# borglab/gtsfm

Measured on NVIDIA H100. Metric: image_pairs_per_sec, higher is better.
Workload: dtype f32

## Files before the change

### gtsfm_b200/csrc/gemm_ws.cuh

```cuda
#pragma once
#include "tma.cuh"

constexpr int GW_MAXP = 16;
constexpr int GW_M = 128, GW_N = 128, GW_K = 64;
constexpr int GW_A_BYTES = GW_M * GW_K * 2;
constexpr int GW_B_BYTES = GW_N * GW_K * 2;
constexpr int GW_STAGE_BYTES = 2 * GW_A_BYTES + 2 * GW_B_BYTES;
constexpr int GW_STAGES = 2;
constexpr int GW_PITCH = GW_N + 8;
constexpr int GW_STG_BYTES = GW_M * GW_PITCH * 4;
constexpr int GW_RB = 8;
constexpr int GW_EW = 4;
constexpr int GW_THREADS = 512;
constexpr size_t GW_SMEM = GW_STAGES * GW_STAGE_BYTES + GW_STG_BYTES + 1024  + 256 ;
constexpr int GW_SEGS = 3;

struct GemmProblem {
  const float* resid;
  float* C;
  __half *Ch[GW_SEGS], *Cl[GW_SEGS];
  const float *cs, *sn;
  int M, N, ldc;
  int vec4;
  int tiles_n;
  int tile_end;
};
struct GemmWsMaps {
  CUtensorMap a1h[GW_MAXP], a1l[GW_MAXP];
  CUtensorMap a2h[GW_MAXP], a2l[GW_MAXP];
  CUtensorMap bh[GW_MAXP], bl[GW_MAXP];
};
struct GemmWsArgs {
  GemmProblem p[GW_MAXP];
  int nprob, tiles;
  int K1, K2;
  int b_per_problem;
  const float* bias;
  int ldr;
  float scale;
  int ldch;
  int head_major;
  int relu;
  int gelu;
  int lo_unscaled;
  int seg_n;
  int rot_mask;
  int* err_flag;
};

static __device__ __noinline__ float gelu_erf(float x) { return 0.5f * x * (1.0f + erff(x * 0.70710678118654752440f)); }

static __global__ void __launch_bounds__(GW_THREADS, 1) k_gemm_ws(const __grid_constant__ GemmWsMaps maps, const __grid_constant__ GemmWsArgs g) {
  extern __shared__ unsigned char gw_raw[];
  const uint32_t raw = tc::smem_u32(gw_raw);
  const uint32_t smem0 = (raw + 1023u) & ~1023u;
  unsigned char* sm = gw_raw + (smem0 - raw);
  float* stg = reinterpret_cast<float*>(sm + GW_STAGES * GW_STAGE_BYTES);
  uint64_t* full = reinterpret_cast<uint64_t*>(sm + GW_STAGES * GW_STAGE_BYTES + GW_STG_BYTES);
  uint64_t* empty = full + GW_STAGES;
  uint64_t* sfull = empty + GW_STAGES;
  uint64_t* sempty = sfull + 1;

  const int t = threadIdx.x, warp = t >> 5, lane = t & 31;
  const int nk = (g.K1 + g.K2) / GW_K;

  if (t == 0) {
    for (int s = 0; s < GW_STAGES; ++s) tc::mbar_init(&full[s], 1), tc::mbar_init(&empty[s], 8);
    tc::mbar_init(sfull, 256);
    tc::mbar_init(sempty, 32 * GW_EW);
    tc::fence_mbar_init();
    tc::tma_prefetch_desc(&maps.bh[0]);
    tc::tma_prefetch_desc(&maps.bl[0]);
  }
  __syncthreads();
  bool ok = true;

  auto decode = [&](int tile, int& z, int& m0, int& n0) {
    z = 0;
    while (z + 1 < g.nprob && tile >= g.p[z].tile_end) ++z;
    const int local = tile - (z ? g.p[z - 1].tile_end : 0);
    const int mt = local / g.p[z].tiles_n;
    n0 = (local - mt * g.p[z].tiles_n) * GW_N;
    m0 = mt * GW_M;
  };

  if (warp >= 12) {
    asm volatile("setmaxnreg.dec.sync.aligned.u32 40;\n" ::: "memory");
    if (warp == 12 && lane == 0) {
      int gk = 0;
      for (int tile = blockIdx.x; tile < g.tiles; tile += gridDim.x) {
        int z, m0, n0;
        decode(tile, z, m0, n0);
        const int zb = g.b_per_problem ? z : 0;
        for (int kc = 0; kc < nk; ++kc, ++gk) {
          const int s = gk % GW_STAGES;
          if (gk >= GW_STAGES) ok = tc::mbar_wait(&empty[s], ((gk / GW_STAGES) - 1) & 1) && ok;
          const int k0 = kc * GW_K;
          const bool seg2 = k0 >= g.K1;
          const CUtensorMap* ah = seg2 ? &maps.a2h[z] : &maps.a1h[z];
          const CUtensorMap* al = seg2 ? &maps.a2l[z] : &maps.a1l[z];
          const int ka = seg2 ? k0 - g.K1 : k0;
          const uint32_t sA = smem0 + s * GW_STAGE_BYTES, sB = sA + 2 * GW_A_BYTES;
          tc::mbar_expect_tx(&full[s], GW_STAGE_BYTES);
          tc::tma_load_2d(sA, ah, &full[s], ka, m0);
          tc::tma_load_2d(sA + GW_A_BYTES, al, &full[s], ka, m0);
          tc::tma_load_2d(sB, &maps.bh[zb], &full[s], k0, n0);
          tc::tma_load_2d(sB + GW_B_BYTES, &maps.bl[zb], &full[s], k0, n0);
        }
      }
    }
  } else if (warp < 8) {
    asm volatile("setmaxnreg.inc.sync.aligned.u32 184;\n" ::: "memory");
    const int wg = warp >> 2;
    const int r0 = wg * 64 + (warp & 3) * 16 + (lane >> 2);
    const int c2 = (lane & 3) * 2;
    int gk = 0, it = 0;
    for (int tile = blockIdx.x; tile < g.tiles; tile += gridDim.x, ++it) {
      float acc0[64], acc1[64];
      for (int kc = 0; kc < nk; ++kc, ++gk) {
        const int s = gk % GW_STAGES;
        ok = tc::mbar_wait(&full[s], (gk / GW_STAGES) & 1) && ok;
        const uint32_t aH = smem0 + s * GW_STAGE_BYTES + wg * (64 * 128), aL = aH + GW_A_BYTES;
        const uint32_t bH = smem0 + s * GW_STAGE_BYTES + 2 * GW_A_BYTES, bL = bH + GW_B_BYTES;
        const uint64_t dAh = tc::wg_desc_sw128(aH), dAl = tc::wg_desc_sw128(aL), dBh = tc::wg_desc_sw128(bH), dBl = tc::wg_desc_sw128(bL);
        tc::wg_fence();
#pragma unroll
        for (int ks = 0; ks < GW_K / 16; ++ks) {
          const uint64_t adv = (uint64_t)(ks * 2);
          const uint32_t first = (kc == 0 && ks == 0) ? 0u : 1u;
          tc::wg_ss_n128(acc0, dAh + adv, dBh + adv, first);
          tc::wg_ss_n128(acc1, dAh + adv, dBl + adv, first);
          tc::wg_ss_n128(acc1, dAl + adv, dBh + adv, 1u);
        }
        tc::wg_commit();
        if (kc > 0) {
          tc::wg_wait<1>();
          if (lane == 0) tc::mbar_arrive(&empty[(gk - 1) % GW_STAGES]);
        }
      }
      tc::wg_wait<0>();
      if (lane == 0) tc::mbar_arrive(&empty[(gk - 1) % GW_STAGES]);

      if (it > 0) ok = tc::mbar_wait(sempty, (it - 1) & 1) && ok;
#pragma unroll
      for (int j = 0; j < 16; ++j)
#pragma unroll
        for (int h = 0; h < 2; ++h) {
          const int i = 4 * j + 2 * h;
          *reinterpret_cast<float2*>(stg + (r0 + 8 * h) * GW_PITCH + 8 * j + c2) =
              make_float2(fmaf(acc1[i], tc::LO_INV, acc0[i]), fmaf(acc1[i + 1], tc::LO_INV, acc0[i + 1]));
        }
      tc::mbar_arrive(sfull);
    }
  } else {
    asm volatile("setmaxnreg.dec.sync.aligned.u32 104;\n" ::: "memory");
    const int ew = warp - 8;
    const int c = 4 * lane;
    const float scale = g.scale;
    const int relu = g.relu, gelu = g.gelu, hm = g.head_major, lo_unscaled = g.lo_unscaled, ldr = g.ldr, ldch = g.ldch;
    int it = 0;
    for (int tile = blockIdx.x; tile < g.tiles; tile += gridDim.x, ++it) {
      int z, m0, n0;
      decode(tile, z, m0, n0);
      const GemmProblem& pb = g.p[z];
      const float* resid = pb.resid;
      float* C = pb.C;
      const int sg = g.seg_n ? n0 / g.seg_n : 0;
      __half *Ch = pb.Ch[sg], *Cl = pb.Cl[sg];
      const bool rot = (g.rot_mask >> sg) & 1;
      const int M = pb.M, ldc = pb.ldc;
      const int n = n0 + c;
      const int ncols = min(4, pb.N - n);
      const bool vec = pb.vec4 && ncols == 4;
      const int rows = min(GW_M, M - m0);
      float b4[4] = {0.f, 0.f, 0.f, 0.f};
      if (g.bias)
#pragma unroll
        for (int e = 0; e < 4; ++e)
          if (e < ncols) b4[e] = __ldg(g.bias + n + e);
      const int ns = n - sg * g.seg_n;
      const size_t hm_col = (size_t)(ns >> 6) * M * 64 + (ns & 63);
      const bool vres = resid && vec;
      const int rp = (ns & 63) >> 1;
      float4 rr[GW_RB];
      auto load_rows = [&](int rb) {
        if (rot) {
#pragma unroll
          for (int i = 0; i < GW_RB; ++i)
            if (rb + GW_EW * i < rows) {
              const size_t o = (size_t)(m0 + rb + GW_EW * i) * 32 + rp;
              const float2 cc = __ldg(reinterpret_cast<const float2*>(pb.cs + o)), ss = __ldg(reinterpret_cast<const float2*>(pb.sn + o));
              rr[i] = make_float4(cc.x, cc.y, ss.x, ss.y);
            }
        } else {
#pragma unroll
          for (int i = 0; i < GW_RB; ++i)
            if (rb + GW_EW * i < rows) rr[i] = *reinterpret_cast<const float4*>(resid + (size_t)(m0 + rb + GW_EW * i) * ldr + n);
        }
      };
      if (vres || rot) load_rows(ew);
      ok = tc::mbar_wait(sfull, it & 1) && ok;
      auto pre = [&](int r, float* v) {
        const float4 a = *reinterpret_cast<const float4*>(stg + r * GW_PITCH + c);
        v[0] = a.x, v[1] = a.y, v[2] = a.z, v[3] = a.w;
#pragma unroll
        for (int e = 0; e < 4; ++e) {
          v[e] = (v[e] + b4[e]) * scale;
          if (relu) v[e] = fmaxf(v[e], 0.f);
          if (gelu) v[e] = gelu_erf(v[e]);
        }
      };
      if (ncols > 0 && vec) {
        for (int rb = ew; rb < rows; rb += GW_EW * GW_RB) {
          if ((vres || rot) && rb != ew) load_rows(rb);
#pragma unroll
          for (int i = 0; i < GW_RB; ++i) {
            const int r = rb + GW_EW * i;
            if (r >= rows) break;
            const int row = m0 + r;
            float v[4];
            pre(r, v);
            if (resid) v[0] += rr[i].x, v[1] += rr[i].y, v[2] += rr[i].z, v[3] += rr[i].w;
            if (rot) {
              const float c0 = rr[i].x, c1 = rr[i].y, s0 = rr[i].z, s1 = rr[i].w;
              const float a0 = __fadd_rn(__fmul_rn(v[0], c0), __fmul_rn(-v[1], s0)), a1 = __fadd_rn(__fmul_rn(v[1], c0), __fmul_rn(v[0], s0));
              const float a2 = __fadd_rn(__fmul_rn(v[2], c1), __fmul_rn(-v[3], s1)), a3 = __fadd_rn(__fmul_rn(v[3], c1), __fmul_rn(v[2], s1));
              v[0] = a0, v[1] = a1, v[2] = a2, v[3] = a3;
            }
            const size_t off = hm ? hm_col + (size_t)row * 64 : (size_t)row * ldc + n;
            if (C) *reinterpret_cast<float4*>(C + off) = make_float4(v[0], v[1], v[2], v[3]);
            if (Ch) {
              const size_t off_s = hm ? off : (size_t)row * ldch + n;
              uint32_t h01, l01, h23, l23;
              if (lo_unscaled) {
                tc::split2_unscaled_clamped(v[0], v[1], h01, l01);
                tc::split2_unscaled_clamped(v[2], v[3], h23, l23);
              } else {
                tc::split2(v[0], v[1], h01, l01);
                tc::split2(v[2], v[3], h23, l23);
              }
              *reinterpret_cast<uint2*>(Ch + off_s) = make_uint2(h01, h23);
              *reinterpret_cast<uint2*>(Cl + off_s) = make_uint2(l01, l23);
            }
          }
        }
      } else if (ncols > 0) {
#pragma unroll 1
        for (int r = ew; r < rows; r += GW_EW) {
          const int row = m0 + r;
          float v[4];
          pre(r, v);
          const size_t off_c = hm ? hm_col + (size_t)row * 64 : (size_t)row * ldc + n;
          const size_t off_s = hm ? hm_col + (size_t)row * 64 : (size_t)row * ldch + n;
#pragma unroll
          for (int e = 0; e < 4; ++e) {
            if (e >= ncols) break;
            if (resid) v[e] += resid[(size_t)row * ldr + n + e];
            if (C) C[off_c + e] = v[e];
            if (Ch) {
              __half hh, ll;
              if (lo_unscaled) tc::split_h_unscaled(v[e], hh, ll);
              else tc::split_h(v[e], hh, ll);
              Ch[off_s + e] = hh;
              Cl[off_s + e] = ll;
            }
          }
        }
      }
      tc::mbar_arrive(sempty);
    }
  }
  if (!ok && g.err_flag) *g.err_flag = 1;
}
```

### gtsfm_b200/csrc/linear.cuh

```cuda
#pragma once
#include "attn_ps.cuh"
#include "common.cuh"
#include "gemm.cuh"
#include "gemm_ws.cuh"

struct TcWeights {
  const float* f;
  const __half* h;
  const __half* l;
  int* err;
  bool use_tc;
  DevBuf* attn_part = nullptr;
  DevBuf* attn_ml = nullptr;
  DevBuf* attn_cnt = nullptr;
  int sm_count = 132;
};

struct Pl {
  __half* hi;
  __half* lo;
};
static inline Pl planes_of(const DevBuf& b, size_t elems) { return {b.as<__half>(), b.as<__half>() + elems}; }

struct LinArgs {
  const float* a1f = nullptr;
  Pl a1p{nullptr, nullptr};
  int lda1 = 0, K1 = 0;
  const float* a2f = nullptr;
  Pl a2p{nullptr, nullptr};
  int lda2 = 0, K2 = 0;
  const float* w = nullptr;
  const float* bf = nullptr;
  Pl bp{nullptr, nullptr};
  int ldb = 0;
  const float* bias = nullptr;
  float scale = 1.f;
  const float* resid = nullptr;
  int ldr = 0;
  float* cf = nullptr;
  int ldc = 0;
  Pl cp{nullptr, nullptr};
  int ldch = 0;
  int head_major = 0;
  bool tc_want_f32 = false;
  int relu = 0;
  int gelu = 0;
  int lo_unscaled = 0;
  int M = 0, N = 0;
  int seg_n = 0;
  float* seg_f[GW_SEGS] = {};
  Pl seg_p[GW_SEGS] = {};
  int rot_mask = 0;
  const float *cs = nullptr, *sn = nullptr;
};

static int run_linear(b2_context* ctx, cudaStream_t st, const TcWeights& tw, const LinArgs* a, int np, const char* site = nullptr) {
  if (np <= 0) return B2_OK;
  if (np > GW_MAXP) return b2_fail(ctx, B2_ERR_ARG, "run_linear: too many problems in one launch");
  const LinArgs& a0 = a[0];
  const int nseg = a0.seg_n > 0 ? a0.N / a0.seg_n : 1;
  if (a0.seg_n > 0 && (a0.seg_n % GW_N || a0.N != nseg * a0.seg_n || nseg > GW_SEGS || !a0.head_major || a0.resid || a0.tc_want_f32 ||
                       (a0.rot_mask && (!a0.cs || !a0.sn))))
    return b2_fail(ctx, B2_ERR_ARG, "run_linear: column segments need N = seg_n x (<= 3), seg_n % 128 == 0, head-major planes, "
                                    "no residual or fp32 output, and a rotary table when rotary is on");
  if (!tw.use_tc) {
    if (a0.rot_mask) return b2_fail(ctx, B2_ERR_ARG, "run_linear: the rotary epilogue exists on the wgmma path only");
    for (int i = 0; i < np; ++i) {
      const LinArgs& x = a[i];
      if (x.M <= 0 || x.N <= 0) continue;
      if (x.gelu) return b2_fail(ctx, B2_ERR_ARG, "run_linear: the GELU epilogue exists on the wgmma path only");
      if (x.K1 % GB_K || x.K2 % GB_K || x.lda1 % 4 || x.lda2 % 4 || x.ldb % 4)
        return b2_fail(ctx, B2_ERR_ARG, "run_linear: the SIMT GEMM needs K1, K2 multiples of 16 and lda1, lda2, ldb multiples of 4");
    }
    for (int i = 0; i < np; ++i) {
      const LinArgs& x = a[i];
      if (x.M <= 0 || x.N <= 0) continue;
      for (int s = 0; s < nseg; ++s) {
        const int c0 = s * x.seg_n;
        GemmArgs g{};
        g.A1 = x.a1f, g.lda1 = x.lda1, g.K1 = x.K1, g.A2 = x.a2f, g.lda2 = x.lda2, g.K2 = x.K2;
        g.B = (x.w ? x.w : x.bf) + (size_t)c0 * x.ldb, g.ldb = x.ldb, g.C = x.seg_n ? x.seg_f[s] : x.cf, g.ldc = x.ldc, g.M = x.M;
        g.N = x.seg_n ? x.seg_n : x.N;
        g.bias = x.bias ? x.bias + c0 : nullptr, g.resid = x.resid, g.ldr = x.ldr, g.scale = x.scale, g.head_major = x.head_major;
        g.relu = x.relu;
        int rc = launch_gemm(ctx, st, g);
        if (rc) return rc;
      }
    }
    return B2_OK;
  }
  if (a0.K1 % GW_K || a0.K2 % GW_K) return b2_fail(ctx, B2_ERR_ARG, "run_linear: the wgmma GEMM needs K1 and K2 multiples of 64");
  if (!tma_encoder()) return b2_fail(ctx, B2_ERR_CUDA, "cuTensorMapEncodeTiled is not available (driver too old?)");
  const bool per_b = a0.w == nullptr;
  static thread_local GemmWsMaps maps;
  GemmWsArgs q{};
  double work = 0.0;
  bool ok = true;
  int nz = 0, tiles = 0;
  for (int i = 0; i < np; ++i) {
    const LinArgs& x = a[i];
    if (x.M <= 0 || x.N <= 0) continue;
    ok = ok && tma_map_2d(&maps.a1h[nz], x.a1p.hi, x.M, x.K1, x.lda1, GW_M) && tma_map_2d(&maps.a1l[nz], x.a1p.lo, x.M, x.K1, x.lda1, GW_M);
    if (x.K2 > 0)
      ok = ok && tma_map_2d(&maps.a2h[nz], x.a2p.hi, x.M, x.K2, x.lda2, GW_M) && tma_map_2d(&maps.a2l[nz], x.a2p.lo, x.M, x.K2, x.lda2, GW_M);
    if (per_b || nz == 0) {
      const __half *bh, *bl;
      if (x.w) {
        const size_t off = (size_t)(x.w - tw.f);
        bh = tw.h + off, bl = tw.l + off;
      } else {
        bh = x.bp.hi, bl = x.bp.lo;
      }
      ok = ok && tma_map_2d(&maps.bh[nz], bh, x.N, x.K1 + x.K2, x.ldb, GW_N) && tma_map_2d(&maps.bl[nz], bl, x.N, x.K1 + x.K2, x.ldb, GW_N);
    }
    GemmProblem& pr = q.p[nz];
    pr.resid = x.resid, pr.C = x.tc_want_f32 ? x.cf : nullptr, pr.M = x.M, pr.N = x.N, pr.ldc = x.ldc;
    for (int s = 0; s < GW_SEGS; ++s) {
      const Pl p = x.seg_n ? (s < nseg ? x.seg_p[s] : Pl{nullptr, nullptr}) : (s == 0 ? x.cp : Pl{nullptr, nullptr});
      pr.Ch[s] = p.hi, pr.Cl[s] = p.lo;
    }
    pr.cs = x.cs, pr.sn = x.sn;
    {
      auto al16 = [](const void* q) { return (reinterpret_cast<uintptr_t>(q) & 15) == 0; };
      auto al8 = [](const void* q) { return (reinterpret_cast<uintptr_t>(q) & 7) == 0; };
      const bool hm = x.head_major != 0;
      bool v = al16(pr.resid) && (x.ldr % 4 == 0 || !pr.resid) && al16(pr.C) && (hm || x.ldc % 4 == 0 || !pr.C);
      v = v && (hm || x.ldch % 4 == 0 || !pr.Ch[0]);
      for (int s = 0; s < GW_SEGS; ++s) v = v && al8(pr.Ch[s]) && al8(pr.Cl[s]);
      v = v && al8(pr.cs) && al8(pr.sn);
      pr.vec4 = v ? 1 : 0;
      if (x.seg_n && !v) return b2_fail(ctx, B2_ERR_ARG, "run_linear: column segments need 8-byte aligned planes and rotary tables");
    }
    pr.tiles_n = cdiv(x.N, GW_N);
    tiles += cdiv(x.M, GW_M) * pr.tiles_n;
    pr.tile_end = tiles;
    work += 2.0 * x.M * x.N * (x.K1 + x.K2);
    ++nz;
  }
  if (nz == 0) return B2_OK;
  if (!ok) return b2_fail(ctx, B2_ERR_CUDA, "cuTensorMapEncodeTiled failed");
  q.nprob = nz, q.tiles = tiles, q.K1 = a0.K1, q.K2 = a0.K2, q.b_per_problem = per_b ? 1 : 0;
  q.bias = a0.bias, q.ldr = a0.ldr, q.scale = a0.scale, q.ldch = a0.ldch;
  q.head_major = a0.head_major, q.relu = a0.relu, q.gelu = a0.gelu, q.lo_unscaled = a0.lo_unscaled, q.err_flag = tw.err;
  q.seg_n = a0.seg_n, q.rot_mask = a0.rot_mask;
  const std::string name = site ? std::string("k_gemm_ws/") + site : std::string("k_gemm_ws");
  b2_prof_work(ctx, name.c_str(), work);
  B2_LAUNCH_NAMED(ctx, name.c_str(), k_gemm_ws, tiles < tw.sm_count ? tiles : tw.sm_count, GW_THREADS, GW_SMEM, st, maps, q);
  B2_CHECK_LAUNCH(ctx);
  return B2_OK;
}

struct FlashPlanes {
  Pl q, k, v, o;
  int nq, nk;
  int heads, ldo;
};
static int run_flash_planes(b2_context* ctx, cudaStream_t st, const TcWeights& tw, const FlashPlanes* jobs, int np, float scale,
                            bool fp16_single = false) {
  if (np <= 0) return B2_OK;
  if (np > AP_MAXP) return b2_fail(ctx, B2_ERR_ARG, "run_flash: too many problems in one launch");
  if (!tma_encoder() || !tw.attn_part) return b2_fail(ctx, B2_ERR_CUDA, "wgmma attention needs cuTensorMapEncodeTiled and its scratch buffers");
  static thread_local AttnPsMaps tmaps;
  AttnPsArgs pa{};
  bool okm = true;
  int items = 0, nz = 0, W = 0, tmax = 0;
  double work = 0.0;
  for (int i = 0; i < np; ++i) {
    const FlashPlanes& j = jobs[i];
    if (j.nq <= 0 || j.nk <= 0) continue;
    AttnPsProblem& p = pa.p[nz];
    p.Qh = j.q.hi, p.Ql = j.q.lo, p.Oh = j.o.hi, p.Ol = j.o.lo, p.Nq = j.nq, p.Nk = j.nk, p.ldo = j.ldo;
    p.qt = cdiv(j.nq, 2 * AW_Q), p.tiles = cdiv(j.nk, AW_KV);
    p.item0 = items;
    items += p.qt * j.heads;
    W += p.qt * j.heads * p.tiles;
    p.w_end = W;
    tmax = p.tiles > tmax ? p.tiles : tmax;
    const uint64_t rows = (uint64_t)j.heads * j.nk;
    okm = okm && tma_map_2d(&tmaps.kh[nz], j.k.hi, rows, 64, 64, AW_KV) && tma_map_2d(&tmaps.kl[nz], j.k.lo, rows, 64, 64, AW_KV);
    okm = okm && tma_map_2d(&tmaps.vh[nz], j.v.hi, rows, 64, 64, AW_KV) && tma_map_2d(&tmaps.vl[nz], j.v.lo, rows, 64, 64, AW_KV);
    work += j.heads * 2.0 * 2.0 * 64 * (double)j.nq * j.nk;
    ++nz;
  }
  if (nz == 0) return B2_OK;
  if (!okm) return b2_fail(ctx, B2_ERR_CUDA, "cuTensorMapEncodeTiled failed (attention)");
  pa.nprob = nz, pa.W = W;
  int ncta = W < tw.sm_count ? W : tw.sm_count;
  pa.quota = cdiv(W, ncta);
  ncta = cdiv(W, pa.quota);
  pa.max_splits = cdiv(tmax, pa.quota) + 1;
  B2_CUDA(ctx, tw.attn_part->ensure((size_t)items * pa.max_splits * 256 * 64 * 4));
  B2_CUDA(ctx, tw.attn_ml->ensure((size_t)items * pa.max_splits * 256 * 2 * 4));
  {
    DevBuf& cnt = *tw.attn_cnt;
    const size_t need = (size_t)items * 2 * sizeof(int);
    if (cnt.cap < need) {
      B2_CUDA(ctx, cnt.ensure(need * 4));
      B2_CUDA(ctx, cudaMemsetAsync(cnt.p, 0, cnt.cap, st));
    }
    pa.arrivals = cnt.as<int>();
  }
  pa.Opart = tw.attn_part->as<float>(), pa.ml = tw.attn_ml->as<float>();
  pa.scale = scale, pa.err_flag = tw.err;
  b2_prof_work(ctx, "k_flash_ps", work);
  if (fp16_single) B2_LAUNCH(ctx, k_flash_ps<true>, ncta, AS_THREADS, AS_SMEM, st, tmaps, pa);
  else B2_LAUNCH(ctx, k_flash_ps<false>, ncta, AS_THREADS, AS_SMEM, st, tmaps, pa);
  B2_CHECK_LAUNCH(ctx);
  return B2_OK;
}

struct FlashJob {
  const DevBuf *q, *k, *v, *o;
  int nq, nk;
  int capq, capk;
};
static int run_flash(b2_context* ctx, cudaStream_t st, const TcWeights& tw, const FlashJob* jobs, int np, float scale, bool fp16_single = false) {
  if (np <= 0) return B2_OK;
  if (np > AP_MAXP) return b2_fail(ctx, B2_ERR_ARG, "run_flash: too many problems in one launch");
  if (!tw.use_tc) {
    for (int i = 0; i < np; ++i) {
      const FlashJob& j = jobs[i];
      int rc = launch_flash(ctx, st, j.q->as<float>(), j.k->as<float>(), j.v->as<float>(), j.o->as<float>(), j.nq, j.nk, scale);
      if (rc) return rc;
    }
    return B2_OK;
  }
  FlashPlanes fp[AP_MAXP];
  for (int i = 0; i < np; ++i) {
    const FlashJob& j = jobs[i];
    fp[i] = {planes_of(*j.q, (size_t)j.capq * 256), planes_of(*j.k, (size_t)j.capk * 256), planes_of(*j.v, (size_t)j.capk * 256),
             planes_of(*j.o, (size_t)j.capq * 256), j.nq, j.nk, 4, 256};
  }
  return run_flash_planes(ctx, st, tw, fp, np, scale, fp16_single);
}
```

Before: 129.7.

## Split GEMM epilogue staging into per-warpgroup halves with 8-wide stores

Staging shared memory is halved to 64 rows, and each MMA warpgroup hands its half to the epilogue warps through its own full/empty barrier pair. This lets epilogue work on one half overlap with the other warpgroup's MMA and store phases. The freed shared memory pays for a third TMA pipeline stage. Epilogue lanes now handle 8 columns each, using 16-byte half-precision stores and float4 rotary/residual loads, with a lane-swizzled read to avoid bank conflicts. The cost is stricter 16-byte alignment requirements and more complex barrier sequencing.

```diff
diff --git a/gtsfm_b200/csrc/gemm_ws.cuh b/gtsfm_b200/csrc/gemm_ws.cuh
--- a/gtsfm_b200/csrc/gemm_ws.cuh
+++ b/gtsfm_b200/csrc/gemm_ws.cuh
@@ -6,11 +6,12 @@
 constexpr int GW_A_BYTES = GW_M * GW_K * 2;
 constexpr int GW_B_BYTES = GW_N * GW_K * 2;
 constexpr int GW_STAGE_BYTES = 2 * GW_A_BYTES + 2 * GW_B_BYTES;
-constexpr int GW_STAGES = 2;
-constexpr int GW_PITCH = GW_N + 8;
-constexpr int GW_STG_BYTES = GW_M * GW_PITCH * 4;
-constexpr int GW_RB = 8;
+constexpr int GW_STAGES = 3;
+constexpr int GW_PITCH = GW_N + 4;
+constexpr int GW_STG_BYTES = 64 * GW_PITCH * 4;
 constexpr int GW_EW = 4;
+constexpr int GW_KH = 64 / (2 * GW_EW);
+constexpr int GW_RB = 4;
 constexpr int GW_THREADS = 512;
 constexpr size_t GW_SMEM = GW_STAGES * GW_STAGE_BYTES + GW_STG_BYTES + 1024  + 256 ;
 constexpr int GW_SEGS = 3;
@@ -21,7 +22,7 @@
   __half *Ch[GW_SEGS], *Cl[GW_SEGS];
   const float *cs, *sn;
   int M, N, ldc;
-  int vec4;
+  int vec8;
   int tiles_n;
   int tile_end;
 };
@@ -59,15 +60,14 @@
   uint64_t* full = reinterpret_cast<uint64_t*>(sm + GW_STAGES * GW_STAGE_BYTES + GW_STG_BYTES);
   uint64_t* empty = full + GW_STAGES;
   uint64_t* sfull = empty + GW_STAGES;
-  uint64_t* sempty = sfull + 1;
+  uint64_t* sempty = sfull + 2;
 
   const int t = threadIdx.x, warp = t >> 5, lane = t & 31;
   const int nk = (g.K1 + g.K2) / GW_K;
 
   if (t == 0) {
     for (int s = 0; s < GW_STAGES; ++s) tc::mbar_init(&full[s], 1), tc::mbar_init(&empty[s], 8);
-    tc::mbar_init(sfull, 256);
-    tc::mbar_init(sempty, 32 * GW_EW);
+    for (int w = 0; w < 2; ++w) tc::mbar_init(&sfull[w], 128), tc::mbar_init(&sempty[w], 32 * GW_EW);
     tc::fence_mbar_init();
     tc::tma_prefetch_desc(&maps.bh[0]);
     tc::tma_prefetch_desc(&maps.bl[0]);
@@ -141,23 +141,27 @@
       tc::wg_wait<0>();
       if (lane == 0) tc::mbar_arrive(&empty[(gk - 1) % GW_STAGES]);
 
-      if (it > 0) ok = tc::mbar_wait(sempty, (it - 1) & 1) && ok;
-#pragma unroll
-      for (int j = 0; j < 16; ++j)
+      if (wg == 1) ok = tc::mbar_wait(&sempty[0], it & 1) && ok;
+      else if (it > 0) ok = tc::mbar_wait(&sempty[1], (it - 1) & 1) && ok;
+#pragma unroll
+      for (int jc = 0; jc < 16; ++jc)
 #pragma unroll
         for (int h = 0; h < 2; ++h) {
-          const int i = 4 * j + 2 * h;
-          *reinterpret_cast<float2*>(stg + (r0 + 8 * h) * GW_PITCH + 8 * j + c2) =
+          const int i = 4 * jc + 2 * h;
+          *reinterpret_cast<float2*>(stg + (r0 - 64 * wg + 8 * h) * GW_PITCH + 8 * jc + c2) =
               make_float2(fmaf(acc1[i], tc::LO_INV, acc0[i]), fmaf(acc1[i + 1], tc::LO_INV, acc0[i + 1]));
         }
-      tc::mbar_arrive(sfull);
+      tc::mbar_arrive(&sfull[wg]);
     }
   } else {
     asm volatile("setmaxnreg.dec.sync.aligned.u32 104;\n" ::: "memory");
     const int ew = warp - 8;
-    const int c = 4 * lane;
+    const int hl = lane >> 4;
+    const int c = 8 * (lane & 15);
+    const int q = (lane >> 2) & 1;
     const float scale = g.scale;
     const int relu = g.relu, gelu = g.gelu, hm = g.head_major, lo_unscaled = g.lo_unscaled, ldr = g.ldr, ldch = g.ldch;
+    auto row_of = [&](int h, int k) { return 64 * h + 2 * (ew + GW_EW * k) + hl; };
     int it = 0;
     for (int tile = blockIdx.x; tile < g.tiles; tile += gridDim.x, ++it) {
       int z, m0, n0;
@@ -170,104 +174,121 @@
       const bool rot = (g.rot_mask >> sg) & 1;
       const int M = pb.M, ldc = pb.ldc;
       const int n = n0 + c;
-      const int ncols = min(4, pb.N - n);
-      const bool vec = pb.vec4 && ncols == 4;
+      const int ncols = min(8, pb.N - n);
+      const bool vec = pb.vec8 && ncols == 8;
       const int rows = min(GW_M, M - m0);
-      float b4[4] = {0.f, 0.f, 0.f, 0.f};
-      if (g.bias)
-#pragma unroll
-        for (int e = 0; e < 4; ++e)
-          if (e < ncols) b4[e] = __ldg(g.bias + n + e);
+      float b8[8];
+#pragma unroll
+      for (int e = 0; e < 8; ++e) b8[e] = g.bias && e < ncols ? __ldg(g.bias + n + e) : 0.f;
       const int ns = n - sg * g.seg_n;
       const size_t hm_col = (size_t)(ns >> 6) * M * 64 + (ns & 63);
       const bool vres = resid && vec;
       const int rp = (ns & 63) >> 1;
-      float4 rr[GW_RB];
-      auto load_rows = [&](int rb) {
+      float4 rr[GW_RB][2];
+      auto load_rows = [&](int h, int k0) {
         if (rot) {
 #pragma unroll
-          for (int i = 0; i < GW_RB; ++i)
-            if (rb + GW_EW * i < rows) {
-              const size_t o = (size_t)(m0 + rb + GW_EW * i) * 32 + rp;
-              const float2 cc = __ldg(reinterpret_cast<const float2*>(pb.cs + o)), ss = __ldg(reinterpret_cast<const float2*>(pb.sn + o));
-              rr[i] = make_float4(cc.x, cc.y, ss.x, ss.y);
-            }
+          for (int i = 0; i < GW_RB; ++i) {
+            const int r = row_of(h, k0 + i);
+            if (r < rows) {
+              const size_t o = (size_t)(m0 + r) * 32 + rp;
+              rr[i][0] = __ldg(reinterpret_cast<const float4*>(pb.cs + o)), rr[i][1] = __ldg(reinterpret_cast<const float4*>(pb.sn + o));
+            }
+          }
         } else {
 #pragma unroll
-          for (int i = 0; i < GW_RB; ++i)
-            if (rb + GW_EW * i < rows) rr[i] = *reinterpret_cast<const float4*>(resid + (size_t)(m0 + rb + GW_EW * i) * ldr + n);
+          for (int i = 0; i < GW_RB; ++i) {
+            const int r = row_of(h, k0 + i);
+            if (r < rows) {
+              const float* src = resid + (size_t)(m0 + r) * ldr + n;
+              rr[i][0] = *reinterpret_cast<const float4*>(src), rr[i][1] = *reinterpret_cast<const float4*>(src + 4);
+            }
+          }
         }
       };
-      if (vres || rot) load_rows(ew);
-      ok = tc::mbar_wait(sfull, it & 1) && ok;
       auto pre = [&](int r, float* v) {
-        const float4 a = *reinterpret_cast<const float4*>(stg + r * GW_PITCH + c);
-        v[0] = a.x, v[1] = a.y, v[2] = a.z, v[3] = a.w;
-#pragma unroll
-        for (int e = 0; e < 4; ++e) {
-          v[e] = (v[e] + b4[e]) * scale;
+        const float* s = stg + (r & 63) * GW_PITCH + c;
+        const float4 x = *reinterpret_cast<const float4*>(s + 4 * q), y = *reinterpret_cast<const float4*>(s + 4 - 4 * q);
+        const float4 a = q ? y : x, b = q ? x : y;
+        v[0] = a.x, v[1] = a.y, v[2] = a.z, v[3] = a.w, v[4] = b.x, v[5] = b.y, v[6] = b.z, v[7] = b.w;
+#pragma unroll
+        for (int e = 0; e < 8; ++e) {
+          v[e] = (v[e] + b8[e]) * scale;
           if (relu) v[e] = fmaxf(v[e], 0.f);
           if (gelu) v[e] = gelu_erf(v[e]);
         }
       };
-      if (ncols > 0 && vec) {
-        for (int rb = ew; rb < rows; rb += GW_EW * GW_RB) {
-          if ((vres || rot) && rb != ew) load_rows(rb);
-#pragma unroll
-          for (int i = 0; i < GW_RB; ++i) {
-            const int r = rb + GW_EW * i;
+      for (int h = 0; h < 2; ++h) {
+        if (vres || rot) load_rows(h, 0);
+        ok = tc::mbar_wait(&sfull[h], it & 1) && ok;
+        if (ncols > 0 && vec) {
+          for (int k0 = 0; k0 < GW_KH && row_of(h, k0) < rows; k0 += GW_RB) {
+            if ((vres || rot) && k0) load_rows(h, k0);
+#pragma unroll
+            for (int i = 0; i < GW_RB; ++i) {
+              const int r = row_of(h, k0 + i);
+              if (r >= rows) break;
+              const int row = m0 + r;
+              float v[8];
+              pre(r, v);
+              if (resid) {
+                v[0] += rr[i][0].x, v[1] += rr[i][0].y, v[2] += rr[i][0].z, v[3] += rr[i][0].w;
+                v[4] += rr[i][1].x, v[5] += rr[i][1].y, v[6] += rr[i][1].z, v[7] += rr[i][1].w;
+              }
+              if (rot) {
+                const float cp[4] = {rr[i][0].x, rr[i][0].y, rr[i][0].z, rr[i][0].w}, sp[4] = {rr[i][1].x, rr[i][1].y, rr[i][1].z, rr[i][1].w};
+#pragma unroll
+                for (int p = 0; p < 4; ++p) {
+                  const float a0 = __fadd_rn(__fmul_rn(v[2 * p], cp[p]), __fmul_rn(-v[2 * p + 1], sp[p]));
+                  const float a1 = __fadd_rn(__fmul_rn(v[2 * p + 1], cp[p]), __fmul_rn(v[2 * p], sp[p]));
+                  v[2 * p] = a0, v[2 * p + 1] = a1;
+                }
+              }
+              const size_t off = hm ? hm_col + (size_t)row * 64 : (size_t)row * ldc + n;
+              if (C) {
+                *reinterpret_cast<float4*>(C + off) = make_float4(v[0], v[1], v[2], v[3]);
+                *reinterpret_cast<float4*>(C + off + 4) = make_float4(v[4], v[5], v[6], v[7]);
+              }
+              if (Ch) {
+                const size_t off_s = hm ? off : (size_t)row * ldch + n;
+                uint32_t hh[4], ll[4];
+#pragma unroll
+                for (int p = 0; p < 4; ++p) {
+                  if (lo_unscaled) tc::split2_unscaled_clamped(v[2 * p], v[2 * p + 1], hh[p], ll[p]);
+                  else tc::split2(v[2 * p], v[2 * p + 1], hh[p], ll[p]);
+                }
+                *reinterpret_cast<uint4*>(Ch + off_s) = make_uint4(hh[0], hh[1], hh[2], hh[3]);
+                *reinterpret_cast<uint4*>(Cl + off_s) = make_uint4(ll[0], ll[1], ll[2], ll[3]);
+              }
+            }
+          }
+        } else if (ncols > 0) {
+#pragma unroll 1
+          for (int k = 0; k < GW_KH; ++k) {
+            const int r = row_of(h, k);
             if (r >= rows) break;
             const int row = m0 + r;
-            float v[4];
+            float v[8];
             pre(r, v);
-            if (resid) v[0] += rr[i].x, v[1] += rr[i].y, v[2] += rr[i].z, v[3] += rr[i].w;
-            if (rot) {
-              const float c0 = rr[i].x, c1 = rr[i].y, s0 = rr[i].z, s1 = rr[i].w;
-              const float a0 = __fadd_rn(__fmul_rn(v[0], c0), __fmul_rn(-v[1], s0)), a1 = __fadd_rn(__fmul_rn(v[1], c0), __fmul_rn(v[0], s0));
-              const float a2 = __fadd_rn(__fmul_rn(v[2], c1), __fmul_rn(-v[3], s1)), a3 = __fadd_rn(__fmul_rn(v[3], c1), __fmul_rn(v[2], s1));
-              v[0] = a0, v[1] = a1, v[2] = a2, v[3] = a3;
-            }
-            const size_t off = hm ? hm_col + (size_t)row * 64 : (size_t)row * ldc + n;
-            if (C) *reinterpret_cast<float4*>(C + off) = make_float4(v[0], v[1], v[2], v[3]);
-            if (Ch) {
-              const size_t off_s = hm ? off : (size_t)row * ldch + n;
-              uint32_t h01, l01, h23, l23;
-              if (lo_unscaled) {
-                tc::split2_unscaled_clamped(v[0], v[1], h01, l01);
-                tc::split2_unscaled_clamped(v[2], v[3], h23, l23);
-              } else {
-                tc::split2(v[0], v[1], h01, l01);
-                tc::split2(v[2], v[3], h23, l23);
-              }
-              *reinterpret_cast<uint2*>(Ch + off_s) = make_uint2(h01, h23);
-              *reinterpret_cast<uint2*>(Cl + off_s) = make_uint2(l01, l23);
-            }
-          }
-        }
-      } else if (ncols > 0) {
-#pragma unroll 1
-        for (int r = ew; r < rows; r += GW_EW) {
-          const int row = m0 + r;
-          float v[4];
-          pre(r, v);
-          const size_t off_c = hm ? hm_col + (size_t)row * 64 : (size_t)row * ldc + n;
-          const size_t off_s = hm ? hm_col + (size_t)row * 64 : (size_t)row * ldch + n;
-#pragma unroll
-          for (int e = 0; e < 4; ++e) {
-            if (e >= ncols) break;
-            if (resid) v[e] += resid[(size_t)row * ldr + n + e];
-            if (C) C[off_c + e] = v[e];
-            if (Ch) {
-              __half hh, ll;
-              if (lo_unscaled) tc::split_h_unscaled(v[e], hh, ll);
-              else tc::split_h(v[e], hh, ll);
-              Ch[off_s + e] = hh;
-              Cl[off_s + e] = ll;
-            }
-          }
-        }
+            const size_t off_c = hm ? hm_col + (size_t)row * 64 : (size_t)row * ldc + n;
+            const size_t off_s = hm ? hm_col + (size_t)row * 64 : (size_t)row * ldch + n;
+#pragma unroll
+            for (int e = 0; e < 8; ++e) {
+              if (e >= ncols) break;
+              if (resid) v[e] += resid[(size_t)row * ldr + n + e];
+              if (C) C[off_c + e] = v[e];
+              if (Ch) {
+                __half hh, ll;
+                if (lo_unscaled) tc::split_h_unscaled(v[e], hh, ll);
+                else tc::split_h(v[e], hh, ll);
+                Ch[off_s + e] = hh;
+                Cl[off_s + e] = ll;
+              }
+            }
+          }
+        }
+        tc::mbar_arrive(&sempty[h]);
       }
-      tc::mbar_arrive(sempty);
     }
   }
   if (!ok && g.err_flag) *g.err_flag = 1;
diff --git a/gtsfm_b200/csrc/linear.cuh b/gtsfm_b200/csrc/linear.cuh
--- a/gtsfm_b200/csrc/linear.cuh
+++ b/gtsfm_b200/csrc/linear.cuh
@@ -122,14 +122,13 @@
     pr.cs = x.cs, pr.sn = x.sn;
     {
       auto al16 = [](const void* q) { return (reinterpret_cast<uintptr_t>(q) & 15) == 0; };
-      auto al8 = [](const void* q) { return (reinterpret_cast<uintptr_t>(q) & 7) == 0; };
       const bool hm = x.head_major != 0;
       bool v = al16(pr.resid) && (x.ldr % 4 == 0 || !pr.resid) && al16(pr.C) && (hm || x.ldc % 4 == 0 || !pr.C);
-      v = v && (hm || x.ldch % 4 == 0 || !pr.Ch[0]);
-      for (int s = 0; s < GW_SEGS; ++s) v = v && al8(pr.Ch[s]) && al8(pr.Cl[s]);
-      v = v && al8(pr.cs) && al8(pr.sn);
-      pr.vec4 = v ? 1 : 0;
-      if (x.seg_n && !v) return b2_fail(ctx, B2_ERR_ARG, "run_linear: column segments need 8-byte aligned planes and rotary tables");
+      v = v && (hm || x.ldch % 8 == 0 || !pr.Ch[0]);
+      for (int s = 0; s < GW_SEGS; ++s) v = v && al16(pr.Ch[s]) && al16(pr.Cl[s]);
+      v = v && al16(pr.cs) && al16(pr.sn);
+      pr.vec8 = v ? 1 : 0;
+      if (x.seg_n && !v) return b2_fail(ctx, B2_ERR_ARG, "run_linear: column segments need 16-byte aligned planes and rotary tables");
     }
     pr.tiles_n = cdiv(x.N, GW_N);
     tiles += cdiv(x.M, GW_M) * pr.tiles_n;
```

Result: faster. 132.6, median of 6 (+2.2%).
